# alexanderswerdlow/unidisc

Hardware: AMD Instinct MI355X
Metric: denoising tokens/sec (fwd+bwd), 1.4B DiT seq_len=1280 (higher is better)
Workload: dtype bf16; 1 GPU; UniDisc 1.4B non-interleaved, seq_len=1280 (256 text + 1024 image), bf16; per_gpu_batch=8, global_batch=8, seq_len=1280, parallelism=dp1, weights=random init (zero_linear_init=false), attention_forward=bf16

## Files before the change

### include/unidisc_hip.h

```cpp
#ifndef UNIDISC_HIP_H
#define UNIDISC_HIP_H

#include <stdint.h>

#ifdef __cplusplus
extern "C" {
#endif

#ifndef __HIP__
typedef struct ihipStream_t* hipStream_t;
#endif

#define UDM_ABI_VERSION 4

#define UDM_EPI_NONE 0
#define UDM_EPI_BIAS 1
#define UDM_EPI_BIAS_GELU 2
#define UDM_EPI_DGELU 3

const char* udm_last_error(void);
int udm_debug_set(const char* key, int64_t value);
int udm_debug_cu_hog(int64_t blocks, const int* flag, hipStream_t stream);
int udm_abi_version(void);

// ... 73 lines not shown
                              int64_t v_stride, int64_t o_stride, int64_t do_stride, int64_t dq_stride, int64_t dk_stride, int64_t dv_stride, int64_t flags, float p_drop,
                              uint64_t seed, hipStream_t stream);

int udm_attention_fwd_kv(const void* q, const void* k, const void* v, void* o, float* lse, int64_t B, int64_t H, int64_t Lq, int64_t Lk, int64_t D, int64_t q_stride,
                         int64_t k_stride, int64_t v_stride, int64_t o_stride, int64_t q_batch, int64_t k_batch, int64_t v_batch, int64_t o_batch, int64_t flags,
                         hipStream_t stream);
int udm_attention_fwd_kv_split(const void* q, const void* k, const void* v, void* o, float* lse, int64_t B, int64_t H, int64_t Lq, int64_t Lk, int64_t D,
                               int64_t q_stride, int64_t k_stride, int64_t v_stride, int64_t o_stride, int64_t q_batch, int64_t k_batch, int64_t v_batch,
                               int64_t o_batch, float* ws, int64_t ws_elems, int64_t splits, int64_t flags, hipStream_t stream);
int udm_attention_kv_split_plan(int64_t B, int64_t H, int64_t Lq, int64_t Lk, int64_t D, int64_t splits, int64_t* splits_out, int64_t* ws_elems_out);

int udm_embedding_fwd(const int64_t* ids, const float* E, const int64_t* modality, const float* Em, float* x, int64_t M, int64_t d, int64_t V,
                      hipStream_t stream);
int udm_embedding_bwd(const int64_t* ids, const int64_t* modality, const float* dx, float* dE, float* dEm, int64_t M, int64_t d, int64_t V, int64_t hot_id,
                      hipStream_t stream);

int udm_subs_ce_fwd(const void* logits, int64_t ld, const int64_t* x0, const int64_t* xt, const int64_t* modality, float* log_p, float* lse, int64_t M,
                    int64_t V, int64_t Vt, int64_t mask_id, int restrict_modality, hipStream_t stream);
int udm_subs_ce_bwd(void* logits, int64_t ld, const int64_t* x0, const int64_t* xt, const int64_t* modality, const float* lse, const float* g, int64_t M,
                    int64_t V, int64_t Vt, int64_t mask_id, int restrict_modality, int64_t narrow_txt_rows, hipStream_t stream);
int udm_subs_logprobs(const void* logits, int64_t ld, const int64_t* xt, const int64_t* modality, void* out, int64_t ld_out, int out_f32, int64_t M, int64_t V,
                      int64_t Vt, int64_t mask_id, int restrict_modality, hipStream_t stream);

int udm_diffusion_loss(const float* log_p, const float* w_loss, const float* w_std, const void* attention_mask, const void* modality_mask, float* nlls, float* coef,
                       float* scalars, int64_t B, int64_t L, int weighted, int full_mask, float text_w, float img_w, float ratio, hipStream_t stream);

int udm_timestep_embedding(const float* sigma, void* out, int64_t B, int64_t dim, hipStream_t stream);
int udm_silu_fwd(const void* x, void* y, int64_t n, hipStream_t stream);
int udm_silu_bwd(const void* x, const void* dy, void* dx, int64_t n, hipStream_t stream);

// ... 74 lines not shown
```

### unidisc_amd/_lib.py

```python
from __future__ import annotations

import ctypes
import os
import subprocess
from ctypes import c_double, c_float, c_int, c_int64, c_uint64, c_void_p

_HERE = os.path.dirname(os.path.abspath(__file__))
LIB_PATH = os.path.join(_HERE, "libunidisc_hip.so")
CSRC = os.path.join(_HERE, "csrc")

_P, _I64, _I, _F, _U64, _D = c_void_p, c_int64, c_int, c_float, c_uint64, c_double

PROTOTYPES = {
    "udm_gemm_nt_bf16": [_P, _P, _P, _I64, _I64, _I64, _I64, _I64, _I64, _I, _I, _P, _P, _I64, _F, _P],
    "udm_gemm_tn_bf16": [_P, _P, _P, _I64, _I64, _I64, _I64, _I64, _I64, _F, _P],
    "udm_gemm_nn_bf16": [_P, _P, _P, _I64, _I64, _I64, _I64, _I64, _I64, _P],
    "udm_gemm_nn_ok": [_I64, _I64, _I64],
    "udm_gemm_nt_splitk_bf16": [_P, _P, _P, _I64, _I64, _I64, _I64, _I64, _I64, _P, _I64, _P],
    "udm_gemm_nn_splitk_bf16": [_P, _P, _P, _I64, _I64, _I64, _I64, _I64, _I64, _P, _I64, _P],
    "udm_gemm_tn_splitk_bf16": [_P, _P, _P, _I64, _I64, _I64, _I64, _I64, _I64, _F, _P, _I64, _P],
    "udm_gemm_tn_pair_bf16": [_P, _P, _P, _I64, _I64, _I64, _I64, _P, _P, _P, _I64, _I64, _I64, _I64, _I64, _I64, _F, _P, _I64, _P],
    "udm_gemm_tn_multi_bf16": [_I, _P, _P, _P, _P, _P, _P, _P, _I64, _F, _P, _I64, _P],
    "udm_gemm_set_cus": [_I],
    "udm_debug_set": [ctypes.c_char_p, _I64],
# ... 31 lines not shown
    "udm_rowgroup_sum_f32": [_P, _P, _P, _I64, _I64, _I64, _P],
    "udm_sample_t_noise": [_P, _I64, _I, _F, _F, _F, _P, _P, _P, _P, _P],
    "udm_qxt_absorbing": [_P, _P, _P, _P, _P, _F, _F, _P, _I64, _I64, _I64, _P, _P, _P, _P, _P, _P],
    "udm_categorical_sample_rows": [_P, _P, _P, _I64, _P, _P, _I64, _U64, _P, _P, _P, _I64, _I64, _I64, _I64, _I, _P],
    "udm_ddpm_sample_rows_cfg": [_P, _P, _P, _I64, _P, _P, _P, _P, _I64, _U64, _P, _I64, _I64, _I64, _I64, _I, _I, _P],
    "udm_ddpm_sample_rows": [_P, _I64, _P, _P, _P, _P, _I64, _U64, _P, _I64, _I64, _I64, _I64, _I, _I, _P],
    "udm_sumsq_f32": [_P, _I64, _P, _P, _I64, _P],
    "udm_adamw_step_ema": [_P, _P, _P, _P, _I64, _F, _D, _D, _F, _F, _I64, _P, _F, _P, _F, _P],
    "udm_adamw_step_shadow_ema": [_P, _P, _P, _P, _I64, _I64, _F, _D, _D, _F, _F, _I64, _P, _F, _P, _I64, _P, _I64, _P, _F, _P],
    "udm_adamw_step_shadow_multi": [_P, _I64, _I64, _F, _D, _D, _F, _F, _I64, _P, _F, _F, _P],
    "udm_adamw_step_multi": [_P, _I64, _I64, _F, _D, _D, _F, _F, _I64, _P, _F, _F, _P],
    "udm_adamw_step": [_P, _P, _P, _P, _I64, _F, _D, _D, _F, _F, _I64, _P, _F, _P],
    "udm_adamw_step_shadow": [_P, _P, _P, _P, _I64, _I64, _F, _D, _D, _F, _F, _I64, _P, _F, _P, _I64, _P, _I64, _P],
    "udm_embedding_fwd": [_P, _P, _P, _P, _P, _I64, _I64, _I64, _P],
    "udm_embedding_bwd": [_P, _P, _P, _P, _P, _I64, _I64, _I64, _I64, _P],
    "udm_subs_ce_fwd": [_P, _I64, _P, _P, _P, _P, _P, _I64, _I64, _I64, _I64, _I, _P],
    "udm_subs_ce_bwd": [_P, _I64, _P, _P, _P, _P, _P, _I64, _I64, _I64, _I64, _I, _I64, _P],
    "udm_subs_logprobs": [_P, _I64, _P, _P, _P, _I64, _I, _I64, _I64, _I64, _I64, _I, _P],
    "udm_subs_logp_rows": [_P, _P, _P, _I64, _P, _P, _P, _I64, _I64, _I64, _I64, _I, _P],
    "udm_likelihood_scores": [_P, _P, _P, _P, _P, _P, _I64, _I64, _I64, _P],
    "udm_diffusion_loss": [_P, _P, _P, _P, _P, _P, _P, _P, _I64, _I64, _I, _I, _F, _F, _F, _P],
    "udm_timestep_embedding": [_P, _P, _I64, _I64, _P],
    "udm_silu_fwd": [_P, _P, _I64, _P],
    "udm_silu_bwd": [_P, _P, _P, _I64, _P],
    "udm_gemm_skinny_bf16": [_P, _P, _P, _I64, _I64, _I64, _I64, _I64, _I64, _I, _I, _P, _P, _I64, _P],
    "udm_attention_decode": [_P, _P, _P, _P, _P, _P, _P, _I64, _I64, _I64, _I64, _I64, _I64, _I64, _I64, _I64, _I64, _P],
    "udm_ar_sample_rows": [_P, _P, _P, _I64, _P, _I64, _P, _I64, _I64, _U64, _I64, _P, _I64, _P, _P, _I64, _P, _I64, _I64, _I64, _I64, _I, _P],
    "udm_nucleus_sample_rows": [_P, _P, _P, _I64, _P, _P, _I64, _U64, _F, _F, _P, _P, _P, _I64, _I64, _I64, _I64, _I, _P],
    "udm_ar_nucleus_rows": [_P, _P, _P, _I64, _P, _I64, _P, _I64, _I64, _U64, _I64, _F, _F, _P, _I64, _P, _P, _I64, _P, _I64, _I64, _I64, _I64, _I, _P],
    "udm_reveal_rows": [_P, _I64, _P, _I64, _P, _P, _P, _I64, _P, _P, _P, _I64, _P, _I64, _U64, _F, _I, _I64, _I64, _P, _I64, _P, _P, _I64, _I64, _I64, _I64, _P],
# ... 63 lines not shown
```

### unidisc_amd/csrc/rowops.hip

```cpp
#include "common.h"
#include "rowops_plan.h"
#include <stdlib.h>
#include <type_traits>
#include "../../include/unidisc_hip.h"

namespace {
using namespace udm;

__device__ __forceinline__ void load8_f32(const float* p, float (&v)[8]) {
  float4 a = *reinterpret_cast<const float4*>(p), b = *reinterpret_cast<const float4*>(p + 4);
  v[0] = a.x; v[1] = a.y; v[2] = a.z; v[3] = a.w; v[4] = b.x; v[5] = b.y; v[6] = b.z; v[7] = b.w;
}
__device__ __forceinline__ void store8_f32(float* p, const float (&v)[8]) {
  *reinterpret_cast<float4*>(p) = make_float4(v[0], v[1], v[2], v[3]);
  *reinterpret_cast<float4*>(p + 4) = make_float4(v[4], v[5], v[6], v[7]);
}
__device__ __forceinline__ void load8_bf16(const bf16_t* p, float (&v)[8]) {
  uint4 u = *reinterpret_cast<const uint4*>(p);
  const uint32_t w[4] = {u.x, u.y, u.z, u.w};
#pragma unroll
  for (int k = 0; k < 4; ++k) {
    v[2 * k] = __uint_as_float(w[k] << 16);
    v[2 * k + 1] = __uint_as_float(w[k] & 0xffff0000u);
  }
// ... 74 lines not shown
      if (c >= a.d) continue;
      float w8[8], o[8];
      load8_f32(a.w + c, w8);
#pragma unroll
      for (int k = 0; k < 8; ++k) o[k] = (v[i][k] - mu) * rs * w8[k];
      if (modulate) {
        float sh[8], sc[8];
        load8_bf16(a.shift + (long)b * a.mod_stride + c, sh);
        load8_bf16(a.scale + (long)b * a.mod_stride + c, sc);
#pragma unroll
        for (int k = 0; k < 8; ++k) o[k] = o[k] * (1.f + sc[k]) + sh[k];
      }
      store8_bf16(a.y + row * a.d + c, o);
    }
  }
}

struct NormBwdArgs {
  const bf16_t* dy;
  const float* x;
  const float* rstd;
  const float* mean;
  const float* w;
  const bf16_t* shift;
  const bf16_t* scale;
  const int64_t* modality;
  const int* any_img;
  float* dx;
  float* dw;
  float* dshift;
// ... 38 lines not shown
    const float rs = a.rstd[row];
    const float mu = a.norm_type ? a.mean[row] : 0.f;
    const int b = (int)(row / a.L);
    const bool modulate = a.shift && (!img_only || a.modality[row] == 1);
    float xh[NCH][8], g[NCH][8];
    float s_g = 0.f, s_gx = 0.f;
#pragma unroll
    for (int i = 0; i < NCH; ++i) {
      const int c = (i * 64 + lane) * 8;
      if (c < a.d) {
        float x8[8], dy8[8], w8[8];
        load8_f32(a.x + row * a.d + c, x8);
        load8_bf16(a.dy + row * a.d + c, dy8);
        load8_f32(a.w + c, w8);
#pragma unroll
        for (int k = 0; k < 8; ++k) xh[i][k] = (x8[k] - mu) * rs;
        if (modulate) {
          float sc[8];
          load8_bf16(a.scale + (long)b * a.mod_stride + c, sc);
#pragma unroll
          for (int k = 0; k < 8; ++k) {
            if (MOD) {
              dsh_acc[i][k] += dy8[k];
              dsc_acc[i][k] += dy8[k] * xh[i][k] * w8[k];
            }
            dy8[k] *= (1.f + sc[k]);
          }
        }
#pragma unroll
        for (int k = 0; k < 8; ++k) {
          dw_acc[i][k] += dy8[k] * xh[i][k];
          g[i][k] = dy8[k] * w8[k];
          s_g += g[i][k];
          s_gx += g[i][k] * xh[i][k];
        }
      } else {
#pragma unroll
        for (int k = 0; k < 8; ++k) { xh[i][k] = 0.f; g[i][k] = 0.f; }
      }
    }
    s_gx = wave_sum(s_gx) / a.d;
    s_g = a.norm_type ? wave_sum(s_g) / a.d : 0.f;
#pragma unroll
    for (int i = 0; i < NCH; ++i) {
      const int c = (i * 64 + lane) * 8;
      if (c >= a.d) continue;
      float o[8];
      if (a.accumulate) load8_f32(a.dx + row * a.d + c, o);
      else {
#pragma unroll
        for (int k = 0; k < 8; ++k) o[k] = 0.f;
      }
#pragma unroll
      for (int k = 0; k < 8; ++k) o[k] += rs * (g[i][k] - s_g - xh[i][k] * s_gx);
      store8_f32(a.dx + row * a.d + c, o);
    }
  }
  __shared__ float red[ROWS_PER_BLOCK][64 * 8 + 8];
#pragma unroll
  for (int i = 0; i < NCH; ++i) {
    block_colsum512(red, dw_acc[i], wave, lane, [&](int t, float s) {
      const int c = i * 512 + t;
      if (c < a.d) {
        if (a.ws) a.ws[(long)blockIdx.x * a.d + c] = s;
        else atomicAdd(a.dw + c, s);
      }
    });
    if (MOD) {
      float* dsh = a.dshift + (long)(blockIdx.x / a.bpb) * a.mod_stride;
// ... 599 lines not shown
      }
      if (dEm) {
        const bool txt = modality[rb + u] == 0;
#pragma unroll
        for (int e = 0; e < 4; ++e) { m0[e] += txt ? gv[e] : 0.f; m1[e] += txt ? 0.f : gv[e]; }
      }
    }
  }
#pragma unroll
  for (int e = 0; e < 4; ++e) {
    if (has_hot && hot[e] != 0.f) atomicAdd(dE + hot_id * d + c + e, hot[e]);
    if (dEm) { atomicAdd(dEm + c + e, m0[e]); atomicAdd(dEm + d + c + e, m1[e]); }
  }
}

__global__ void timestep_embedding_kernel(const float* __restrict__ sigma, bf16_t* __restrict__ out, int B, int dim) {
  const int i = blockIdx.x * blockDim.x + threadIdx.x;
  const int half = dim / 2;
  if (i >= B * dim) return;
  const int b = i / dim, j = i % dim;
  float v = 0.f;
  if (j < 2 * half) {
    const int jj = j < half ? j : j - half;
    const float f = expf(-logf(10000.f) * (float)jj / (float)half);
    const float arg = sigma[b] * f;
    v = j < half ? cosf(arg) : sinf(arg);
  }
  out[i] = f2bf(v);
}

// ... 500 lines not shown
    if ((which == 1 && !a.w_b) || (which == 2 && !a.dbias)) continue;
#pragma unroll
    for (int i = 0; i < NCH; ++i) {
      __syncthreads();
#pragma unroll
      for (int k = 0; k < 8; ++k) red[wave][lane * 8 + k] = which == 0 ? dwn[i][k] : (which == 1 ? dwb[i][k] : dbs[i][k]);
      __syncthreads();
      for (int t = threadIdx.x; t < 512; t += 256) {
        const int c = i * 512 + t;
        if (c < a.d) a.ws[((long)blockIdx.x * 3 + which) * a.d + c] = red[0][t] + red[1][t] + red[2][t] + red[3][t];
      }
    }
  }
}

__global__ __launch_bounds__(256) void colreduce3_kernel(const float* __restrict__ ws, float* __restrict__ out0, float* __restrict__ out1, float* __restrict__ out2,
                                                         int nrows, int d) {
  __shared__ float red[4][64];
  const int which = blockIdx.z;
  float* const outp = which == 0 ? out0 : (which == 1 ? out1 : out2);
  if (!outp) return;
  const int col = blockIdx.x * 64 + (threadIdx.x & 63), sub = threadIdx.x >> 6;
  const int per = (nrows + gridDim.y - 1) / gridDim.y;
  const int r0 = blockIdx.y * per, r1 = min(nrows, r0 + per);
  const float* base = ws + (long)which * d;
  const long rstride = 3L * d;
  float s = 0.f;
  if (col < d) {
    float s0 = 0.f, s1 = 0.f, s2 = 0.f, s3 = 0.f;
    int r = r0 + sub;
    for (; r + 12 < r1; r += 16) {
      s0 += base[(long)r * rstride + col];
      s1 += base[(long)(r + 4) * rstride + col];
      s2 += base[(long)(r + 8) * rstride + col];
      s3 += base[(long)(r + 12) * rstride + col];
    }
    for (; r < r1; r += 4) s0 += base[(long)r * rstride + col];
    s = (s0 + s1) + (s2 + s3);
  }
  red[sub][threadIdx.x & 63] = s;
  __syncthreads();
// ... 306 lines not shown
        }
      }
    }
  }
}

template <int... Ns, typename F>
bool with_inst(int inst, F&& f) { return ((inst == Ns && (f(std::integral_constant<int, Ns>{}), true)) || ...); }

template <typename A>
void launch_rows(void (*kernel)(A), const RowPlan& p, hipStream_t stream, const A& a) { hipLaunchKernelGGL(kernel, dim3(p.grid), dim3(256), p.lds_bytes, stream, a); }

int unsupported_width(const char* kernel) { udm_set_error("%s: unsupported hidden size (d <= 2048 or d == 4096, d %% 8 == 0)", kernel); return 2; }

int reduce_rows(const char* launched, const char* reduced, const RowPlan& p, hipStream_t stream, const float* ws, float* out0, int planes = 1, float* out1 = nullptr,
                float* out2 = nullptr) {
  UDM_CHECK_LAUNCH(launched);
  if (!p.use_ws) return 0;
  const dim3 grid((p.reduce_cols + 63) / 64, 16, planes);
  if (planes == 3) hipLaunchKernelGGL(colreduce3_kernel, grid, dim3(256), 0, stream, ws, out0, out1, out2, (int)p.reduce_rows, (int)p.reduce_cols);
  else hipLaunchKernelGGL(colreduce_kernel, grid, dim3(256), 0, stream, ws, out0, (int)p.reduce_rows, (int)p.reduce_cols);
  UDM_CHECK_LAUNCH(reduced);
  return 0;
}

int residual_fwd(const char* name, bool next, bool ada, const float* x_in, const void* branch, float* x_out, const float* w_b, float* rstd_b, float* mean_b,
                 const void* gate, int64_t mod_stride, const int64_t* modality, int64_t M, int64_t d, int64_t L, int norm_type, float eps, float p_drop, uint64_t seed,
                 const float* w_next, void* h_out, float* rstd_next, float* mean_next, const void* next_shift, const void* next_scale, int64_t next_mod_stride,
                 const int64_t* next_modality, const int* next_any_img, hipStream_t stream) {
  UDM_CHECK_ARG(x_in && branch && x_out && (!next || (w_next && h_out && rstd_next)) && (!ada || (next_shift && next_scale)), "%s: null pointer", name);
  UDM_CHECK_ARG(M > 0 && d > 0 && d % 8 == 0 && L > 0, "%s: bad shape", name);
  UDM_CHECK_ARG(!w_b || rstd_b, "%s: sandwich norm needs rstd buffer", name);
  UDM_CHECK_ARG(!(w_b && norm_type) || mean_b, "%s: sandwich LayerNorm needs mean buffer", name);
  UDM_CHECK_ARG(!next || !norm_type || mean_next, "%s: LayerNorm needs mean_next", name);
  UDM_CHECK_ARG(p_drop >= 0.f && p_drop < 1.f, "%s: dropout p out of range", name);
// ... 295 lines not shown

extern "C" int udm_embedding_bwd(const int64_t* ids, const int64_t* modality, const float* dx, float* dE, float* dEm, int64_t M, int64_t d, int64_t V,
                                 int64_t hot_id, hipStream_t stream) {
  UDM_CHECK_ARG(ids && dx && dE, "udm_embedding_bwd: null pointer");
  UDM_CHECK_ARG(M > 0 && d > 0 && V > 0, "udm_embedding_bwd: bad shape");
  UDM_CHECK_ARG(!dEm || modality, "udm_embedding_bwd: modality embedding grad needs the modality map");
  UDM_CHECK_ARG(d % 4 == 0 && ((uintptr_t)dx % 16 == 0), "udm_embedding_bwd: d must be a multiple of 4 and dx 16-byte aligned");
  const int rows_per_block = 128;
  const int grid = (int)((M + rows_per_block - 1) / rows_per_block);
  hipLaunchKernelGGL(embedding_bwd_kernel, dim3(grid, (unsigned)((d + 1023) / 1024)), dim3(256), 0, stream, ids, modality, dx, dE, dEm, (long)M, (int)d, (long)V,
                     (long)hot_id, rows_per_block);
  UDM_CHECK_LAUNCH("udm_embedding_bwd");
  return 0;
}

extern "C" int udm_timestep_embedding(const float* sigma, void* out, int64_t B, int64_t dim, hipStream_t stream) {
  UDM_CHECK_ARG(sigma && out && B > 0 && dim > 0, "udm_timestep_embedding: bad argument");
  const long n = B * dim;
  hipLaunchKernelGGL(timestep_embedding_kernel, dim3((unsigned)((n + 255) / 256)), dim3(256), 0, stream, sigma, (bf16_t*)out, (int)B, (int)dim);
  UDM_CHECK_LAUNCH("udm_timestep_embedding");
  return 0;
}
extern "C" int udm_silu_fwd(const void* x, void* y, int64_t n, hipStream_t stream) {
  UDM_CHECK_ARG(x && y && n > 0, "udm_silu_fwd: bad argument");
  hipLaunchKernelGGL(silu_fwd_kernel, dim3((unsigned)((n + 255) / 256)), dim3(256), 0, stream, (const bf16_t*)x, (bf16_t*)y, (long)n);
  UDM_CHECK_LAUNCH("udm_silu_fwd");
  return 0;
}
extern "C" int udm_silu_bwd(const void* x, const void* dy, void* dx, int64_t n, hipStream_t stream) {
  UDM_CHECK_ARG(x && dy && dx && n > 0, "udm_silu_bwd: bad argument");
// ... 24 lines not shown
```

### unidisc_amd/csrc/rowops_plan.h

```cpp
#pragma once
#include <stdint.h>

constexpr int ROWS_PER_BLOCK = 4;

enum RowForm { WAVE_ROW, BLOCK_ROW, BLOCK_ROW_2ROWS };
struct RowPlan {
  RowForm form = WAVE_ROW;
  int inst = 0;
  uint32_t grid = 0;
  int bpb = 0;
  bool use_ws = false;
  uint32_t lds_bytes = 0;
  uint32_t reduce_rows = 0, reduce_cols = 0;
  long ws_need = 0;
  bool ok = false;
};

constexpr int ROW_GRID_MAX = 2048;
constexpr int ROW_WS_MIN_GRID = 64;
constexpr int NORM_BWD_GRID_NARROW = 1024, NORM_BWD_GRID_WIDE = 512;
constexpr int NORM_BWD_GRID_ATOMICS = 512;
constexpr int RESID_BWD_GRID_GATED = 1024;
constexpr int RESID_BWD_GRID_D2048 = 1024;
constexpr int RESID_BWD_GRID_BROW = 1536;
// ... 52 lines not shown
  }
  const int inst = d < 2048 ? nch_for(d) : 0;
  if (sandwich && grid_rows(M) >= RESID_BWD_GRID_WS && ws_elems >= RESID_BWD_GRID_WS * d) return row_plan_ws(row_plan(WAVE_ROW, inst, RESID_BWD_GRID_WS), d);
  return row_plan(WAVE_ROW, inst, row_min(grid_rows(M), RESID_BWD_GRID));
}
inline RowPlan row_plan_norm_residual_bwd(long M, long d) {
  if (M <= 0 || !(d == 2048 || d == 4096 || (d % 8 == 0 && d >= 64 && d < 2048))) return RowPlan{};
  if (d < 2048) return row_plan_ws(row_plan(WAVE_ROW, nch_for(d), row_min(grid_rows(M), FUSED_BWD_GRID_WROW)), d, 3);
  return row_plan_ws(row_plan(BLOCK_ROW, d == 2048 ? 1 : 2, row_min(M, FUSED_BWD_GRID_BROW)), d, 3);
}
inline RowPlan row_plan_norm_residual_bwd_ada(long M, long d, long L) {
  if (M <= 0 || L <= 0 || M % L != 0 || !(d == 2048 || d == 4096)) return RowPlan{};
  const int bpb = row_bpb(FUSED_ADA_GRID, M / L, L);
  return row_plan_ws(row_plan(BLOCK_ROW, d == 2048 ? 1 : 2, M / L * bpb, bpb), d, 6);
}
inline int qk_nit(long d) { return (int)((2 * (d / 16) + 63) / 64); }
inline bool qk_shape_ok(long d) { return d > 0 && d % 16 == 0 && qk_nit(d) <= 8; }
inline RowPlan row_plan_qk_fwd(long M, long d, bool qk_norm) {
  if (!qk_shape_ok(d)) return RowPlan{};
  const long lds = qk_norm ? 4 * d * (long)sizeof(float) : 0;
  if (d == 2048) return row_plan(BLOCK_ROW_2ROWS, 2, row_min((M + 1) / 2, QK_FWD_GRID_2ROWS));
  if (d > 2048) return row_plan(BLOCK_ROW, 2, row_min(M, QK_FWD_GRID_BROW), 0, lds);
  return row_plan(WAVE_ROW, qk_nit(d), row_min(grid_rows(M), QK_FWD_GRID_WROW), 0, lds);
}
inline RowPlan row_plan_qk_bwd(long M, long d, bool qk_norm, bool contiguous, long ws_elems) {
  if (!qk_shape_ok(d)) return RowPlan{};
  const bool ws_form = qk_norm && contiguous;
  if (d >= 2048) {
    const long g = row_min(M, QK_BWD_GRID_BROW), lds = qk_norm ? 2 * d * (long)sizeof(float) : 0;
    if (ws_form && ws_elems >= g * 4 * d) return row_plan_ws(row_plan(BLOCK_ROW, d <= 2048 ? 1 : 2, g, 0, lds), 4 * d);
// ... 7 lines not shown
```

### unidisc_amd/dit.py

```python
from __future__ import annotations

import math
import types
import os
from dataclasses import dataclass
from typing import Dict, List, Optional

import weakref

import torch
import torch.nn as nn

from . import kernels as K
from .rope import lumina_rope_2d, rotary_table_1d

try:
    from huggingface_hub import PyTorchModelHubMixin as _HubMixin
except Exception:
    class _HubMixin:
        pass

BF16, F32 = torch.bfloat16, torch.float32


# ... 292 lines not shown
            DDiTBlock(d, H, self.cond_dim, dropout=self.dropout, time_conditioning=self.time_conditioning, norm_type=self.norm_type,
                      sandwich_normalization=self.sandwich_normalization, qk_norm=self.qk_norm) for _ in range(self.n_blocks)
        ])
        self.output_layer = DDitFinalLayer(d, vocab_size, self.cond_dim, time_conditioning=self.time_conditioning, norm_type=self.norm_type,
                                           zero_linear_init=cfg_get(m, "zero_linear_init", True))
        self.allow_compiled_embed = False
        if device is not None:
            self.to(device)
        self._lins: Optional[Dict[str, _Lin]] = None
        self._fwd_count = 0
        self.compact_head = True
        self.compact_last_block = os.environ.get("UDM_COMPACT_LAST", "1") != "0"
        self.split_head = os.environ.get("UDM_SPLIT_HEAD", "1") != "0"
        self.pair_wgrads = os.environ.get("UDM_PAIR_WGRADS", "1") != "0"
        self.multi_wgrads = os.environ.get("UDM_MULTI_WGRADS", "1") != "0"
        self.dgrad_from_w = os.environ.get("UDM_DGRAD_NN", "1") != "0"
        self.grad_ready_callback = None
        self.grad_sync_finish = None
        self.recast_every_forward = True
        self.overlap_weight_cast = os.environ.get("UDM_OVERLAP_CAST", "0") != "0"
        self._shadow_versions = None

    def _register_rotary_tables(self, linear_factor):
        D = self.head_dim
        if self.rope_2d:
            if not (self.multimodal_batches and self.modality_embed is not None):
                raise NotImplementedError("unidisc_amd.DIT: rope_2d needs multimodal_batches and modality_embed (as in every shipped config)")
            if self.require_sample_ids:
                for n_img, lf in self.IMG_BLOCKS:
                    side = int(math.sqrt(n_img))
# ... 914 lines not shown
            bp.dc = torch.zeros((S.Bp, self.cond_dim), dtype=F32, device=dev)
            dmodf = torch.zeros((S.Bp, 2 * d), dtype=F32, device=dev)
            if S.Bp <= K.SMALL_BATCH_LINEAR_MAX_B and self.cond_dim <= K.SMALL_BATCH_LINEAR_MAX_IN and self.cond_dim % 8 == 0:
                tiles = K.small_batch_linear_bwd_tiles(2 * d) + self.n_blocks * K.small_batch_linear_bwd_tiles(6 * d)
                bp.ada_buf = torch.empty((tiles, S.Bp, self.cond_dim), dtype=F32, device=dev)
        bp.dx = torch.empty((dhf.shape[0] if S.stream_compact else M, d), dtype=F32, device=dev)
        bp.tc_fused = tc and not S.stream_compact and K.norm_residual_bwd_ada_ok(M, d, S.L)
        pn = _PendingNorm(dy=dhf, x=S.x_final, rstd=S.rstdf, mean=S.meanf, w=fl.norm_final.weight.detach(), dw=G[id(fl.norm_final.weight)], accumulate=False,
                          mod=S.fmod, dmod=dmodf, mod_idx=(0, 1), finish=self.n_blocks)
        if tc:
            self._norm_backward(bp, pn)
        else:
            bp.pend = pn
        for i in reversed(range(self.n_blocks)):
            self._block_backward(bp, i)
        if bp.pend is not None:
            self._norm_backward(bp, bp.pend)
        dx = bp.dx
        if S.cnt_j is not None:
            n_cnt = self.img_count_embedding.shape[0]
            if dx.is_cuda and dx.dtype == F32:
                K.rowgroup_sum(dx, S.cnt_j, G[id(self.img_count_embedding)])
            else:
                gext = torch.zeros((n_cnt + 1, dx.shape[1]), dtype=dx.dtype, device=dx.device).index_add_(0, S.cnt_j, dx)
                G[id(self.img_count_embedding)].add_(gext[:n_cnt])
        K.embedding_bwd(S.ids, dx, G[id(self.vocab_embed.embedding)], self.mask_index, modality=S.emb_mod if self.modality_embed is not None else None,
                        dEm=G[id(self.modality_embed.embedding)] if self.modality_embed is not None else None)
        tail = list(self.vocab_embed.parameters()) + (list(self.modality_embed.parameters()) if self.modality_embed is not None else [])
        if getattr(self, "img_count_embedding", None) is not None:
            tail.append(self.img_count_embedding)
        if tc:
            self._sigma_map_backward(bp)
            tail += list(self.sigma_map.parameters())
        self._notify(bp.flat, tail)
        if self.grad_sync_finish is not None:
            self.grad_sync_finish()
        self._last_grad_flat_ref, self._last_grad_numel = weakref.ref(bp.flat), sum(p.numel() for p in params)
        return [G[id(p)] for p in params]

    def _head_backward(self, bp, grad_out, mode):
        S, G, head = bp.S, bp.G, self._lins["head"]
        M, d, V, dev = S.B * S.L, self.hidden_size, self.vocab_size, S.ids.device
        logits, head_rows, groups = S.logits, S.head_rows, S.head_groups if mode == "logp" else None
# ... 34 lines not shown
                elif c_al:
                    Gw[:c_al].zero_()
                if n_ip:
                    K.gemm_nt_splitk(dlogits[n_tp:, c_al:], head.w16t[:, c_al:], N=d, out=dhf[n_tp:])
                    K.colsum(dlogits[n_tp:, c_al:], db[c_al:])
                    K.gemm_tn(dlogits[n_tp:, c_up:V], hf_h[n_tp:], Gw[c_up:], M=V - c_up, N=d)
                else:
                    Gw[c_up:].zero_()
                if c_up > c_al:
                    K.gemm_tn(dlogits[:, c_al:c_up], hf_h, Gw[c_al:c_up], M=c_up - c_al, N=d)
                G[id(head.bias)].copy_(db[:V])
            else:
                dhf = K.gemm_nt_splitk(dlogits, head.w16t, N=d, out=torch.empty((M, d), dtype=BF16, device=dev)[: dlogits.shape[0]])
                self._wgrad(dlogits, S.hf, head, G)
        if head_rows is not None and not S.stream_compact:
            dhf = torch.zeros((M, d), dtype=dhf.dtype, device=dev).index_copy_(0, head_rows[0], dhf)
        S.logits = None
        return dhf

    def _finish_block(self, bp, i, dmod=None):
        if i is None:
            return
        if dmod is not None:
            self._ada_backward(bp, dmod, self._lins[f"{i}.ada" if i < self.n_blocks else "head.ada"])
        if i < self.n_blocks:
            bp.S.blocks[i] = None
        self._notify(bp.flat, list((self.blocks[i] if i < self.n_blocks else self.output_layer).parameters()))

    def _norm_backward(self, bp, pn):
        S, ada = bp.S, pn.mod is not None
        K.norm_bwd(pn.dy, pn.x, pn.rstd, pn.mean, pn.w, bp.nt, S.L, bp.dx, pn.dw, accumulate=pn.accumulate, mod=pn.mod, dmod=pn.dmod, mod_idx=pn.mod_idx,
# ... 49 lines not shown
        if multi is None:
            self._wgrad(du1, R.h2, f1, G, bias_done=True)
        del du1, du2
        p2 = _PendingNorm(dy=dh2, x=R.x_mid, rstd=R.rstd2, mean=R.mean2, w=blk.norm2.weight.detach(), dw=G[id(blk.norm2.weight)], accumulate=True,
                          mod=mod, dmod=dmod, mod_idx=(3, 4))
        if sw:
            da = self._norm_branch_bwd(bp, p2, R.a_out, w_b=blk.pre_residual_norm.weight.detach(), rstd=R.rstd_a, mean=R.mean_a, norm_type=nt,
                                       dw_b=G[id(blk.pre_residual_norm.weight)])
        elif tc:
            da = self._norm_branch_bwd(bp, p2, R.a_out, mod=mod, dmod=dmod, gate_idx=2, p_drop=p_drop, seed=seed0 + 4 * i + 1)
        else:
            da = self._norm_branch_bwd(bp, p2, R.a_out, p_drop=p_drop, seed=seed0 + 4 * i + 1)
        do = lo.dgrad(da, da.shape[0], S.dgrad_form.get(f"{i}.out"))
        if R.rows_c is not None:
            self._wgrad(da, R.o_c, lo, G)
            do = torch.zeros((M, d), dtype=do.dtype, device=dev).index_copy_(0, R.rows_c, do)
            bp.dx = torch.zeros((M, d), dtype=F32, device=dev).index_copy_(0, R.rows_c, bp.dx)
        elif multi is not None:
            multi.append((da, R.o, lo))
        elif (self.pair_wgrads and da.is_cuda and lo.bias is None and lq.bias is None and lo.inp == lq.inp
                and K.gemm_tn_pair_ok(lq.out, lo.out, lq.inp, M)
                and ((lq.out // 256 + lo.out // 256) * (lq.inp // 256) % 256 == 0 or (lq.out // 256 + lo.out // 256) * (lq.inp // 256) <= 128)):
            pair_out = (da, R.o)
        else:
            self._wgrad(da, R.o, lo, G)
        dqkr, dqkv = torch.empty((M, 2 * d), dtype=BF16, device=dev), torch.empty((M, 3 * d), dtype=BF16, device=dev)
        K.attention_bwd(R.qkr, R.qkv, R.o, do, R.lse, dqkr, dqkv, B, L, H, D, S.sid, S.doc_ranges, q_prescaled=True, **self._attn_mask_kw, **S.attn_drop_kw(i))
        qn = self.qk_norm
        K.qknorm_rope_bwd(dqkr, R.qkv, dqkv, S.cos, S.sin, L, D, gq=at.q_norm.weight.detach() if qn else None, gk=at.k_norm.weight.detach() if qn else None,
                          stats=R.qstats, dgq=G[id(at.q_norm.weight)] if qn else None, dbq=G[id(at.q_norm.bias)] if qn else None,
                          dgk=G[id(at.k_norm.weight)] if qn else None, dbk=G[id(at.k_norm.bias)] if qn else None, q_scale=self.attn_q_scale)
        dh1 = lq.dgrad(dqkv, dqkv.shape[0], S.dgrad_form.get(f"{i}.qkv"))
# ... 59 lines not shown
```

### unidisc_amd/kernels.py

```python
from __future__ import annotations

from typing import Optional

import os

import math

import torch

from . import _lib

EPI_NONE, EPI_BIAS, EPI_BIAS_GELU, EPI_DGELU = 0, 1, 2, 3
NORM_RMS, NORM_LN = 0, 1
BF16, F32 = torch.bfloat16, torch.float32


def _p(t: Optional[torch.Tensor]):
    if t is None:
        return None
    if not t.is_cuda:
        raise RuntimeError("unidisc_amd kernels need GPU tensors (no CPU fallback); got a tensor on " + str(t.device))
    return t.data_ptr()


# ... 517 lines not shown
    return y


def cast_bf16_f32(x, y, scale=1.0):
    _lib.call("udm_cast_bf16_f32", _p(x), _p(y), x.numel(), float(scale), _s())
    return y


_ADA_GRID_ROWS = 768
ROWOPS_WS = {
    "norm_bwd": lambda M, d: 1024 * d if M >= 2048 else 0,
    "residual_bwd": lambda M, d: 1536 * d,
    "norm_residual_bwd": lambda M, d: min(M, 1536) * 3 * d,
    "norm_residual_bwd_ada": lambda M, d: _ADA_GRID_ROWS * 6 * d,
    "qknorm_rope_bwd": lambda M, d: 4096 * d,
}


def norm_residual_bwd_fused_ok(d):
    return d in (2048, 4096) or (d < 2048 and d % 8 == 0 and d >= 64)


def _mod_ptrs(mod, idx, d):
    if mod is None:
        return [None] * len(idx), 0
    es = mod.element_size()
    return [mod.data_ptr() + es * k * d for k in idx], mod.stride(0)


def norm_fwd(x, w, norm_type, L, *, mod=None, mod_idx=(0, 1), modality=None, any_img=None, out=None):
# ... 265 lines not shown

def embedding_fwd(ids, E, modality=None, Em=None, out=None):
    M = ids.numel()
    V, d = E.shape
    x = torch.empty((M, d), dtype=F32, device=E.device) if out is None else out
    _lib.call("udm_embedding_fwd", _p(ids), _p(E), _p(modality), _p(Em), _p(x), M, d, V, _s())
    return x


def embedding_bwd(ids, dx, dE, hot_id, modality=None, dEm=None):
    M = ids.numel()
    V, d = dE.shape
    _lib.call("udm_embedding_bwd", _p(ids), _p(modality), _p(dx), _p(dE), _p(dEm), M, d, V, hot_id, _s())


def subs_ce_fwd(logits, x0, xt, modality, V, Vt, mask_id, restrict):
    M, ld = logits.shape[0], logits.stride(0)
    log_p = torch.empty(M, dtype=F32, device=logits.device)
    lse = torch.empty(M, dtype=F32, device=logits.device)
    _lib.call("udm_subs_ce_fwd", _p(logits), ld, _p(x0), _p(xt), _p(modality), _p(log_p), _p(lse), M, V, Vt, mask_id, 1 if restrict else 0, _s())
    return log_p, lse


def subs_ce_bwd(logits, x0, xt, modality, lse, g, V, Vt, mask_id, restrict, narrow_txt_rows=-1):
    M, ld = logits.shape[0], logits.stride(0)
    _lib.call("udm_subs_ce_bwd", _p(logits), ld, _p(x0), _p(xt), _p(modality), _p(lse), _p(g), M, V, Vt, mask_id, 1 if restrict else 0,
              int(narrow_txt_rows) if restrict else -1, _s())


def subs_logprobs(logits, xt, modality, V, Vt, mask_id, restrict, out_dtype=BF16):
# ... 210 lines not shown
```

Baseline: 129,500 tokens/s.

## Fuse final norm backward with embedding backward and add zero-filling row scatter

Adds a kernel that runs the final norm backward and scatters its per-row gradient straight into the vocab embedding gradient with atomics. It also reduces the hot mask-token and modality embedding gradients through the same workspace column reduction. This removes a separate embedding-backward pass and an extra read of the fp32 dx buffer. It also replaces the torch zeros+index_copy pattern with a single scatter kernel that writes either the source row or zero, and the inverse map is reused for the second scatter. The cost is more atomics contention and shared-memory pressure, and float summation order changes slightly.

```diff
diff --git a/include/unidisc_hip.h b/include/unidisc_hip.h
--- a/include/unidisc_hip.h
+++ b/include/unidisc_hip.h
@@ -111,6 +111,11 @@
                       hipStream_t stream);
 int udm_embedding_bwd(const int64_t* ids, const int64_t* modality, const float* dx, float* dE, float* dEm, int64_t M, int64_t d, int64_t V, int64_t hot_id,
                       hipStream_t stream);
+int udm_norm_embedding_bwd(const void* dy, const float* x, const float* rstd, const float* mean, const float* w, const float* dx, float* dw, int64_t M,
+                           int64_t d, int norm_type, int accumulate, const int64_t* ids, const int64_t* modality, float* dE, float* dEm, int64_t V,
+                           int64_t hot_id, float* ws, int64_t ws_elems, hipStream_t stream);
+int udm_scatter_rows_zero(const void* src, const int64_t* rows, int64_t n_sel, void* dst, int64_t M, int64_t d, int64_t elem_size, int* inv,
+                          int build_inv, hipStream_t stream);
 
 int udm_subs_ce_fwd(const void* logits, int64_t ld, const int64_t* x0, const int64_t* xt, const int64_t* modality, float* log_p, float* lse, int64_t M,
                     int64_t V, int64_t Vt, int64_t mask_id, int restrict_modality, hipStream_t stream);
diff --git a/unidisc_amd/_lib.py b/unidisc_amd/_lib.py
--- a/unidisc_amd/_lib.py
+++ b/unidisc_amd/_lib.py
@@ -69,6 +69,8 @@
     "udm_adamw_step_shadow": [_P, _P, _P, _P, _I64, _I64, _F, _D, _D, _F, _F, _I64, _P, _F, _P, _I64, _P, _I64, _P],
     "udm_embedding_fwd": [_P, _P, _P, _P, _P, _I64, _I64, _I64, _P],
     "udm_embedding_bwd": [_P, _P, _P, _P, _P, _I64, _I64, _I64, _I64, _P],
+    "udm_norm_embedding_bwd": [_P, _P, _P, _P, _P, _P, _P, _I64, _I64, _I, _I, _P, _P, _P, _P, _I64, _I64, _P, _I64, _P],
+    "udm_scatter_rows_zero": [_P, _P, _I64, _P, _I64, _I64, _I64, _P, _I, _P],
     "udm_subs_ce_fwd": [_P, _I64, _P, _P, _P, _P, _P, _I64, _I64, _I64, _I64, _I, _P],
     "udm_subs_ce_bwd": [_P, _I64, _P, _P, _P, _P, _P, _I64, _I64, _I64, _I64, _I, _I64, _P],
     "udm_subs_logprobs": [_P, _I64, _P, _P, _P, _I64, _I, _I64, _I64, _I64, _I64, _I, _P],
diff --git a/unidisc_amd/csrc/rowops.hip b/unidisc_amd/csrc/rowops.hip
--- a/unidisc_amd/csrc/rowops.hip
+++ b/unidisc_amd/csrc/rowops.hip
@@ -112,6 +112,22 @@
       store8_bf16(a.y + row * a.d + c, o);
     }
   }
+}
+
+__device__ __forceinline__ float norm_xhat(float x, float mu, float rs) {
+#pragma clang fp contract(off)
+  return (x - mu) * rs;
+}
+__device__ __forceinline__ void norm_bwd_sums(float dy, float xh, float w, float& dw, float& g, float& s_g, float& s_gx) {
+#pragma clang fp contract(off)
+  dw = __builtin_fmaf(dy, xh, dw);
+  g = dy * w;
+  s_g = s_g + g;
+  s_gx = __builtin_fmaf(g, xh, s_gx);
+}
+__device__ __forceinline__ float norm_bwd_dx(float o, float rs, float g, float s_g, float xh, float s_gx) {
+#pragma clang fp contract(off)
+  return __builtin_fmaf(rs, __builtin_fmaf(-xh, s_gx, g - s_g), o);
 }
 
 struct NormBwdArgs {
@@ -180,7 +196,7 @@
         load8_bf16(a.dy + row * a.d + c, dy8);
         load8_f32(a.w + c, w8);
 #pragma unroll
-        for (int k = 0; k < 8; ++k) xh[i][k] = (x8[k] - mu) * rs;
+        for (int k = 0; k < 8; ++k) xh[i][k] = norm_xhat(x8[k], mu, rs);
         if (modulate) {
           float sc[8];
           load8_bf16(a.scale + (long)b * a.mod_stride + c, sc);
@@ -194,12 +210,7 @@
           }
         }
 #pragma unroll
-        for (int k = 0; k < 8; ++k) {
-          dw_acc[i][k] += dy8[k] * xh[i][k];
-          g[i][k] = dy8[k] * w8[k];
-          s_g += g[i][k];
-          s_gx += g[i][k] * xh[i][k];
-        }
+        for (int k = 0; k < 8; ++k) norm_bwd_sums(dy8[k], xh[i][k], w8[k], dw_acc[i][k], g[i][k], s_g, s_gx);
       } else {
 #pragma unroll
         for (int k = 0; k < 8; ++k) { xh[i][k] = 0.f; g[i][k] = 0.f; }
@@ -218,7 +229,7 @@
         for (int k = 0; k < 8; ++k) o[k] = 0.f;
       }
 #pragma unroll
-      for (int k = 0; k < 8; ++k) o[k] += rs * (g[i][k] - s_g - xh[i][k] * s_gx);
+      for (int k = 0; k < 8; ++k) o[k] = norm_bwd_dx(o[k], rs, g[i][k], s_g, xh[i][k], s_gx);
       store8_f32(a.dx + row * a.d + c, o);
     }
   }
@@ -848,6 +859,117 @@
   }
 }
 
+struct NormEmbBwdArgs {
+  const bf16_t* dy; const float* x; const float* rstd; const float* mean; const float* w;
+  const float* dx;
+  const int64_t* ids;
+  const int64_t* modality;
+  float* dE;
+  float* ws;
+  long V, hot_id;
+  int M, d, norm_type, accumulate;
+};
+
+template <int NCH>
+__global__ __launch_bounds__(256, NCH <= 4 ? 2 : 1) void norm_embedding_bwd_kernel(NormEmbBwdArgs a) {
+  const int lane = threadIdx.x & 63, wave = threadIdx.x >> 6;
+  const bool has_hot = a.hot_id >= 0 && a.hot_id < a.V;
+  __shared__ __attribute__((aligned(16))) float tr[ROWS_PER_BLOCK][NCH * 512];
+  float dw_acc[NCH][8], hot[NCH][8], m0[NCH][8], m1[NCH][8];
+#pragma unroll
+  for (int i = 0; i < NCH; ++i)
+#pragma unroll
+    for (int k = 0; k < 8; ++k) { dw_acc[i][k] = 0.f; hot[i][k] = 0.f; m0[i][k] = 0.f; m1[i][k] = 0.f; }
+  for (long row = (long)blockIdx.x * ROWS_PER_BLOCK + wave; row < a.M; row += (long)gridDim.x * ROWS_PER_BLOCK) {
+    const float rs = a.rstd[row];
+    const float mu = a.norm_type ? a.mean[row] : 0.f;
+    const long id = a.ids[row];
+    const bool is_hot = has_hot && id == a.hot_id, ordinary = !is_hot && id >= 0 && id < a.V;
+    const bool txt = a.modality && a.modality[row] == 0;
+    float xh[NCH][8], g[NCH][8], o[NCH][8];
+    float s_g = 0.f, s_gx = 0.f;
+#pragma unroll
+    for (int i = 0; i < NCH; ++i) {
+      const int c = (i * 64 + lane) * 8;
+      if (c < a.d) {
+        float x8[8], dy8[8], w8[8];
+        load8_f32(a.x + row * a.d + c, x8);
+        load8_bf16(a.dy + row * a.d + c, dy8);
+        load8_f32(a.w + c, w8);
+#pragma unroll
+        for (int k = 0; k < 8; ++k) xh[i][k] = norm_xhat(x8[k], mu, rs);
+#pragma unroll
+        for (int k = 0; k < 8; ++k) norm_bwd_sums(dy8[k], xh[i][k], w8[k], dw_acc[i][k], g[i][k], s_g, s_gx);
+      } else {
+#pragma unroll
+        for (int k = 0; k < 8; ++k) { xh[i][k] = 0.f; g[i][k] = 0.f; }
+      }
+    }
+    s_gx = wave_sum(s_gx) / a.d;
+    s_g = a.norm_type ? wave_sum(s_g) / a.d : 0.f;
+#pragma unroll
+    for (int i = 0; i < NCH; ++i) {
+      const int c = (i * 64 + lane) * 8;
+      if (c >= a.d) continue;
+      if (a.accumulate) load8_f32(a.dx + row * a.d + c, o[i]);
+      else {
+#pragma unroll
+        for (int k = 0; k < 8; ++k) o[i][k] = 0.f;
+      }
+#pragma unroll
+      for (int k = 0; k < 8; ++k) o[i][k] = norm_bwd_dx(o[i][k], rs, g[i][k], s_g, xh[i][k], s_gx);
+      if (is_hot) {
+#pragma unroll
+        for (int k = 0; k < 8; ++k) hot[i][k] += o[i][k];
+      } else if (ordinary) {
+        store8_f32(&tr[wave][c], o[i]);
+      }
+      if (a.modality) {
+#pragma unroll
+        for (int k = 0; k < 8; ++k) { m0[i][k] += txt ? o[i][k] : 0.f; m1[i][k] += txt ? 0.f : o[i][k]; }
+      }
+    }
+    if (ordinary) {
+      float* e = a.dE + id * a.d;
+      __builtin_amdgcn_wave_barrier();
+#pragma unroll 8
+      for (int j = 0; j < NCH * 8; ++j) {
+        const int col = j * 64 + lane;
+        if (col < a.d) atomicAdd(e + col, tr[wave][col]);
+      }
+      __builtin_amdgcn_wave_barrier();
+    }
+  }
+  __shared__ float red[ROWS_PER_BLOCK][64 * 8 + 8];
+  float* const wrow = a.ws + (long)blockIdx.x * 4 * a.d;
+#pragma unroll
+  for (int i = 0; i < NCH; ++i) {
+    block_colsum512(red, dw_acc[i], wave, lane, [&](int t, float s) { if (i * 512 + t < a.d) wrow[i * 512 + t] = s; });
+    if (has_hot) block_colsum512(red, hot[i], wave, lane, [&](int t, float s) { if (i * 512 + t < a.d) wrow[a.d + i * 512 + t] = s; });
+    if (a.modality) {
+      block_colsum512(red, m0[i], wave, lane, [&](int t, float s) { if (i * 512 + t < a.d) wrow[2 * a.d + i * 512 + t] = s; });
+      block_colsum512(red, m1[i], wave, lane, [&](int t, float s) { if (i * 512 + t < a.d) wrow[3 * a.d + i * 512 + t] = s; });
+    }
+  }
+}
+
+__global__ __launch_bounds__(256) void scatter_mark_kernel(const int64_t* __restrict__ rows, int* __restrict__ inv, long n_sel, long M) {
+  const long j = (long)blockIdx.x * 256 + threadIdx.x;
+  if (j >= n_sel) return;
+  const long r = rows[j];
+  if (r >= 0 && r < M) inv[r] = (int)j;
+}
+
+__global__ __launch_bounds__(256) void scatter_rows_zero_kernel(const uint4* __restrict__ src, const int* __restrict__ inv, uint4* __restrict__ dst, long M, int row_vecs,
+                                                                long n_sel) {
+  const long total = M * row_vecs;
+  for (long v = (long)blockIdx.x * 256 + threadIdx.x; v < total; v += (long)gridDim.x * 256) {
+    const long r = v / row_vecs;
+    const int j = inv[r];
+    dst[v] = (j >= 0 && j < n_sel) ? src[(long)j * row_vecs + (v - r * row_vecs)] : make_uint4(0u, 0u, 0u, 0u);
+  }
+}
+
 __global__ void timestep_embedding_kernel(const float* __restrict__ sigma, bf16_t* __restrict__ out, int B, int dim) {
   const int i = blockIdx.x * blockDim.x + threadIdx.x;
   const int half = dim / 2;
@@ -1378,17 +1500,18 @@
   }
 }
 
-__global__ __launch_bounds__(256) void colreduce3_kernel(const float* __restrict__ ws, float* __restrict__ out0, float* __restrict__ out1, float* __restrict__ out2,
-                                                         int nrows, int d) {
+struct ColOuts { float* out[4]; };
+template <int P>
+__global__ __launch_bounds__(256) void colreduce_planes_kernel(const float* __restrict__ ws, ColOuts o, int nrows, int d) {
   __shared__ float red[4][64];
   const int which = blockIdx.z;
-  float* const outp = which == 0 ? out0 : (which == 1 ? out1 : out2);
+  float* const outp = o.out[which];
   if (!outp) return;
   const int col = blockIdx.x * 64 + (threadIdx.x & 63), sub = threadIdx.x >> 6;
   const int per = (nrows + gridDim.y - 1) / gridDim.y;
   const int r0 = blockIdx.y * per, r1 = min(nrows, r0 + per);
   const float* base = ws + (long)which * d;
-  const long rstride = 3L * d;
+  const long rstride = (long)P * d;
   float s = 0.f;
   if (col < d) {
     float s0 = 0.f, s1 = 0.f, s2 = 0.f, s3 = 0.f;
@@ -1725,11 +1848,13 @@
 int unsupported_width(const char* kernel) { udm_set_error("%s: unsupported hidden size (d <= 2048 or d == 4096, d %% 8 == 0)", kernel); return 2; }
 
 int reduce_rows(const char* launched, const char* reduced, const RowPlan& p, hipStream_t stream, const float* ws, float* out0, int planes = 1, float* out1 = nullptr,
-                float* out2 = nullptr) {
+                float* out2 = nullptr, float* out3 = nullptr) {
   UDM_CHECK_LAUNCH(launched);
   if (!p.use_ws) return 0;
   const dim3 grid((p.reduce_cols + 63) / 64, 16, planes);
-  if (planes == 3) hipLaunchKernelGGL(colreduce3_kernel, grid, dim3(256), 0, stream, ws, out0, out1, out2, (int)p.reduce_rows, (int)p.reduce_cols);
+  const ColOuts outs{{out0, out1, out2, out3}};
+  if (planes == 4) hipLaunchKernelGGL(colreduce_planes_kernel<4>, grid, dim3(256), 0, stream, ws, outs, (int)p.reduce_rows, (int)p.reduce_cols);
+  else if (planes == 3) hipLaunchKernelGGL(colreduce_planes_kernel<3>, grid, dim3(256), 0, stream, ws, outs, (int)p.reduce_rows, (int)p.reduce_cols);
   else hipLaunchKernelGGL(colreduce_kernel, grid, dim3(256), 0, stream, ws, out0, (int)p.reduce_rows, (int)p.reduce_cols);
   UDM_CHECK_LAUNCH(reduced);
   return 0;
@@ -2055,6 +2180,43 @@
   return 0;
 }
 
+extern "C" int udm_norm_embedding_bwd(const void* dy, const float* x, const float* rstd, const float* mean, const float* w, const float* dx, float* dw, int64_t M,
+                                      int64_t d, int norm_type, int accumulate, const int64_t* ids, const int64_t* modality, float* dE, float* dEm, int64_t V,
+                                      int64_t hot_id, float* ws, int64_t ws_elems, hipStream_t stream) {
+  const RowPlan plan = row_plan_norm_embedding_bwd(M, d);
+  UDM_CHECK_ARG(dy && x && rstd && w && dw && ids && dE && ws, "udm_norm_embedding_bwd: null pointer");
+  UDM_CHECK_ARG(plan.ok && V > 0, "udm_norm_embedding_bwd: bad shape (M > 0, V > 0, d <= 4096, d %% 8 == 0; got M=%ld d=%ld V=%ld)", (long)M, (long)d, (long)V);
+  UDM_CHECK_ARG(!accumulate || dx, "udm_norm_embedding_bwd: accumulate needs the gradient accumulated so far");
+  UDM_CHECK_ARG(norm_type == 0 || mean, "udm_norm_embedding_bwd: LayerNorm needs the saved mean");
+  UDM_CHECK_ARG(!dEm || modality, "udm_norm_embedding_bwd: modality embedding grad needs the modality map");
+  UDM_CHECK_ARG(ws_elems >= plan.ws_need, "udm_norm_embedding_bwd: workspace too small (need %ld floats)", plan.ws_need);
+  const bool has_hot = hot_id >= 0 && hot_id < V;
+  NormEmbBwdArgs a{(const bf16_t*)dy, x, rstd, mean, w, dx, ids, dEm ? modality : nullptr, dE, ws, (long)V, (long)hot_id, (int)M, (int)d, norm_type, accumulate};
+  (void)with_inst<1, 2, 3, 4, 8>(plan.inst, [&](auto n) { launch_rows(norm_embedding_bwd_kernel<decltype(n)::value>, plan, stream, a); });
+  return reduce_rows("udm_norm_embedding_bwd", "udm_norm_embedding_bwd(colreduce)", plan, stream, ws, dw, NORM_EMB_PLANES, has_hot ? dE + hot_id * d : nullptr,
+                     dEm, dEm ? dEm + d : nullptr);
+}
+
+extern "C" int udm_scatter_rows_zero(const void* src, const int64_t* rows, int64_t n_sel, void* dst, int64_t M, int64_t d, int64_t elem_size, int* inv,
+                                     int build_inv, hipStream_t stream) {
+  UDM_CHECK_ARG(dst && inv && (n_sel == 0 || (src && rows)), "udm_scatter_rows_zero: null pointer");
+  UDM_CHECK_ARG(M > 0 && d > 0 && n_sel >= 0 && n_sel <= M && M * d < (1L << 40), "udm_scatter_rows_zero: bad shape M=%ld d=%ld n_sel=%ld", (long)M, (long)d, (long)n_sel);
+  UDM_CHECK_ARG((elem_size == 2 || elem_size == 4) && (d * elem_size) % 16 == 0 && (uintptr_t)src % 16 == 0 && (uintptr_t)dst % 16 == 0,
+                "udm_scatter_rows_zero: bf16 / fp32 rows of a multiple of 16 bytes, 16-byte aligned");
+  if (build_inv) {
+    if (hipMemsetAsync(inv, 0xff, (size_t)M * sizeof(int), stream) != hipSuccess) { udm_set_error("udm_scatter_rows_zero: memset failed"); return 1; }
+    if (n_sel > 0) {
+      hipLaunchKernelGGL(scatter_mark_kernel, dim3((unsigned)((n_sel + 255) / 256)), dim3(256), 0, stream, rows, inv, (long)n_sel, (long)M);
+      UDM_CHECK_LAUNCH("udm_scatter_rows_zero(mark)");
+    }
+  }
+  const long row_bytes = d * elem_size;
+  hipLaunchKernelGGL(scatter_rows_zero_kernel, dim3((unsigned)scatter_rows_grid(M, row_bytes)), dim3(256), 0, stream, (const uint4*)src, (const int*)inv, (uint4*)dst,
+                     (long)M, (int)(row_bytes / 16), (long)n_sel);
+  UDM_CHECK_LAUNCH("udm_scatter_rows_zero");
+  return 0;
+}
+
 extern "C" int udm_timestep_embedding(const float* sigma, void* out, int64_t B, int64_t dim, hipStream_t stream) {
   UDM_CHECK_ARG(sigma && out && B > 0 && dim > 0, "udm_timestep_embedding: bad argument");
   const long n = B * dim;
diff --git a/unidisc_amd/csrc/rowops_plan.h b/unidisc_amd/csrc/rowops_plan.h
--- a/unidisc_amd/csrc/rowops_plan.h
+++ b/unidisc_amd/csrc/rowops_plan.h
@@ -90,6 +90,17 @@
   const int bpb = row_bpb(FUSED_ADA_GRID, M / L, L);
   return row_plan_ws(row_plan(BLOCK_ROW, d == 2048 ? 1 : 2, M / L * bpb, bpb), d, 6);
 }
+constexpr int NORM_EMB_PLANES = 4;
+inline RowPlan row_plan_norm_embedding_bwd(long M, long d) {
+  if (M <= 0 || d <= 0 || d % 8 != 0 || nch_dispatch(d) == 0) return RowPlan{};
+  const long grid = row_min(grid_rows(M), d < 2048 ? NORM_BWD_GRID_NARROW : NORM_BWD_GRID_WIDE);
+  return row_plan_ws(row_plan(WAVE_ROW, nch_dispatch(d), grid), d, NORM_EMB_PLANES);
+}
+constexpr int SCATTER_GRID_MAX = 8192;
+inline long scatter_rows_grid(long M, long row_bytes) {
+  const long blocks = (M * (row_bytes / 16) + 255) / 256;
+  return blocks < 1 ? 1 : row_min(blocks, SCATTER_GRID_MAX);
+}
 inline int qk_nit(long d) { return (int)((2 * (d / 16) + 63) / 64); }
 inline bool qk_shape_ok(long d) { return d > 0 && d % 16 == 0 && qk_nit(d) <= 8; }
 inline RowPlan row_plan_qk_fwd(long M, long d, bool qk_norm) {
diff --git a/unidisc_amd/dit.py b/unidisc_amd/dit.py
--- a/unidisc_amd/dit.py
+++ b/unidisc_amd/dit.py
@@ -330,6 +330,7 @@
         self.split_head = os.environ.get("UDM_SPLIT_HEAD", "1") != "0"
         self.pair_wgrads = os.environ.get("UDM_PAIR_WGRADS", "1") != "0"
         self.multi_wgrads = os.environ.get("UDM_MULTI_WGRADS", "1") != "0"
+        self.fused_tail = os.environ.get("UDM_FUSED_TAIL", "1") != "0"
         self.dgrad_from_w = os.environ.get("UDM_DGRAD_NN", "1") != "0"
         self.grad_ready_callback = None
         self.grad_sync_finish = None
@@ -1274,8 +1275,16 @@
             bp.pend = pn
         for i in reversed(range(self.n_blocks)):
             self._block_backward(bp, i)
-        if bp.pend is not None:
-            self._norm_backward(bp, bp.pend)
+        pn, emb_mod = bp.pend, self.modality_embed is not None
+        emb_kw = dict(modality=S.emb_mod if emb_mod else None, dEm=G[id(self.modality_embed.embedding)] if emb_mod else None)
+        fused = (pn is not None and self.fused_tail and self.n_blocks > 0 and pn.finish == 0 and pn.mod is None and S.cnt_j is None and bp.dx.is_cuda
+                 and bp.dx.dtype == F32 and K.norm_embedding_bwd_ok(M, d))
+        if fused:
+            K.norm_embedding_bwd(pn.dy, pn.x, pn.rstd, pn.mean, pn.w, bp.nt, bp.dx, pn.dw, S.ids, G[id(self.vocab_embed.embedding)], self.mask_index,
+                                 accumulate=pn.accumulate, **emb_kw)
+            self._finish_block(bp, pn.finish, pn.dmod)
+        elif pn is not None:
+            self._norm_backward(bp, pn)
         dx = bp.dx
         if S.cnt_j is not None:
             n_cnt = self.img_count_embedding.shape[0]
@@ -1284,9 +1293,9 @@
             else:
                 gext = torch.zeros((n_cnt + 1, dx.shape[1]), dtype=dx.dtype, device=dx.device).index_add_(0, S.cnt_j, dx)
                 G[id(self.img_count_embedding)].add_(gext[:n_cnt])
-        K.embedding_bwd(S.ids, dx, G[id(self.vocab_embed.embedding)], self.mask_index, modality=S.emb_mod if self.modality_embed is not None else None,
-                        dEm=G[id(self.modality_embed.embedding)] if self.modality_embed is not None else None)
-        tail = list(self.vocab_embed.parameters()) + (list(self.modality_embed.parameters()) if self.modality_embed is not None else [])
+        if not fused:
+            K.embedding_bwd(S.ids, dx, G[id(self.vocab_embed.embedding)], self.mask_index, **emb_kw)
+        tail = list(self.vocab_embed.parameters()) + (list(self.modality_embed.parameters()) if emb_mod else [])
         if getattr(self, "img_count_embedding", None) is not None:
             tail.append(self.img_count_embedding)
         if tc:
@@ -1351,7 +1360,10 @@
                 dhf = K.gemm_nt_splitk(dlogits, head.w16t, N=d, out=torch.empty((M, d), dtype=BF16, device=dev)[: dlogits.shape[0]])
                 self._wgrad(dlogits, S.hf, head, G)
         if head_rows is not None and not S.stream_compact:
-            dhf = torch.zeros((M, d), dtype=dhf.dtype, device=dev).index_copy_(0, head_rows[0], dhf)
+            if self.fused_tail and dhf.is_cuda:
+                dhf = K.scatter_rows_zero(dhf, head_rows[0], M)[0]
+            else:
+                dhf = torch.zeros((M, d), dtype=dhf.dtype, device=dev).index_copy_(0, head_rows[0], dhf)
         S.logits = None
         return dhf
 
@@ -1431,8 +1443,12 @@
         do = lo.dgrad(da, da.shape[0], S.dgrad_form.get(f"{i}.out"))
         if R.rows_c is not None:
             self._wgrad(da, R.o_c, lo, G)
-            do = torch.zeros((M, d), dtype=do.dtype, device=dev).index_copy_(0, R.rows_c, do)
-            bp.dx = torch.zeros((M, d), dtype=F32, device=dev).index_copy_(0, R.rows_c, bp.dx)
+            if self.fused_tail and do.is_cuda:
+                do, inv = K.scatter_rows_zero(do, R.rows_c, M)
+                bp.dx, _ = K.scatter_rows_zero(bp.dx, R.rows_c, M, inv)
+            else:
+                do = torch.zeros((M, d), dtype=do.dtype, device=dev).index_copy_(0, R.rows_c, do)
+                bp.dx = torch.zeros((M, d), dtype=F32, device=dev).index_copy_(0, R.rows_c, bp.dx)
         elif multi is not None:
             multi.append((da, R.o, lo))
         elif (self.pair_wgrads and da.is_cuda and lo.bias is None and lq.bias is None and lo.inp == lq.inp
diff --git a/unidisc_amd/kernels.py b/unidisc_amd/kernels.py
--- a/unidisc_amd/kernels.py
+++ b/unidisc_amd/kernels.py
@@ -555,6 +555,7 @@
     "norm_residual_bwd": lambda M, d: min(M, 1536) * 3 * d,
     "norm_residual_bwd_ada": lambda M, d: _ADA_GRID_ROWS * 6 * d,
     "qknorm_rope_bwd": lambda M, d: 4096 * d,
+    "norm_embedding_bwd": lambda M, d: 4096 * d,
 }
 
 
@@ -850,6 +851,33 @@
     _lib.call("udm_embedding_bwd", _p(ids), _p(modality), _p(dx), _p(dE), _p(dEm), M, d, V, hot_id, _s())
 
 
+def norm_embedding_bwd_ok(M, d):
+    return M > 0 and 0 < d <= 4096 and d % 8 == 0
+
+
+def norm_embedding_bwd(dy, x, rstd, mean, w, norm_type, dx, dw, ids, dE, hot_id, *, accumulate=True, modality=None, dEm=None):
+    M, d = x.shape
+    V = dE.shape[0]
+    ws = _scratch(ROWOPS_WS["norm_embedding_bwd"](M, d), x.device)
+    _lib.call("udm_norm_embedding_bwd", _p(dy), _p(x), _p(rstd), _p(mean), _p(w), _p(dx) if accumulate else None, _p(dw), M, d, norm_type, 1 if accumulate else 0,
+              _p(ids), _p(modality) if dEm is not None else None, _p(dE), _p(dEm), V, hot_id, _p(ws), ws.numel(), _s())
+
+
+def scatter_rows_zero(src, rows, M, inv=None):
+    n_sel, d = src.shape
+    _chk(rows, torch.int64, "scatter_rows_zero: rows")
+    if not (src.is_contiguous() and rows.is_contiguous() and rows.numel() == n_sel and n_sel <= M):
+        raise ValueError(f"scatter_rows_zero: contiguous src [n_sel, d] and rows [n_sel <= M]; got src {tuple(src.shape)} stride {src.stride()}, rows {tuple(rows.shape)}, M {M}")
+    if __debug__ and os.environ.get("UDM_DEBUG_CHECKS"):
+        assert rows.numel() == n_sel and torch.unique(rows).numel() == n_sel and (n_sel == 0 or (int(rows.min()) >= 0 and int(rows.max()) < M))
+    out = torch.empty((M, d), dtype=src.dtype, device=src.device)
+    build = inv is None
+    if build:
+        inv = torch.empty(M, dtype=torch.int32, device=src.device)
+    _lib.call("udm_scatter_rows_zero", _p(src) if n_sel else None, _p(rows) if n_sel else None, n_sel, _p(out), M, d, src.element_size(), _p(inv), 1 if build else 0, _s())
+    return out, inv
+
+
 def subs_ce_fwd(logits, x0, xt, modality, V, Vt, mask_id, restrict):
     M, ld = logits.shape[0], logits.stride(0)
     log_p = torch.empty(M, dtype=F32, device=logits.device)
```

Result: no change. 129,900 tokens/s, median of 6 (+0.2%).
